# SomeBottle/LinearProgramming

Hardware: AMD Instinct MI355X
Metric: Simplex pivots/sec + HBM GB/s fraction, dense m=16384×n=32768 fp64, 1/2/4/8 GPU (higher is better)
Workload: dtype f64

## Files before the change

### linearprogramming_amd/csrc/lpg_ctx.hip

```cpp
#include <hip/hip_runtime.h>
#include <rccl/rccl.h>

#include <dlfcn.h>
#include <unistd.h>
#include <math.h>
#include <stdarg.h>
#include <stdio.h>
#include <stdlib.h>
#include <string.h>

#include <algorithm>
#include <vector>

#include "../../include/lpg.h"
#include "lpg_internal.h"

using namespace lpg;

namespace {

thread_local char g_err[512];

struct TimingRing {
    std::vector<hipEvent_t> ev;
// ... 205 lines not shown
        const RcclApi *R = rccl_api();
        ncclResult_t r = R->AllReduce(buf, buf, count, ncclFloat64, ncclSum, c->nccl, c->stream);
        if (r != ncclSuccess) return fail(c, LPG_ERR_COMM, "ncclAllReduce: %s", R->GetErrorString(r));
        return 0;
    }
    if (!c->have_hops) return fail(c, LPG_ERR_STATE, "world > 1 but no communicator attached");
    c->hsend.resize(count * sizeof(double));
    HIPCHK(c, hipMemcpyAsync(c->hsend.data(), buf, count * sizeof(double), hipMemcpyDeviceToHost, c->stream));
    HIPCHK(c, hipStreamSynchronize(c->stream));
    if (c->hops.allreduce_sum_f64(c->hops.user, (double *)c->hsend.data(), count) != 0)
        return fail(c, LPG_ERR_COMM, "host allreduce callback failed");
    HIPCHK(c, hipMemcpyAsync(buf, c->hsend.data(), count * sizeof(double), hipMemcpyHostToDevice, c->stream));
    HIPCHK(c, hipStreamSynchronize(c->stream));
    return 0;
}


static int timing_flush(lpg_ctx *c) {
    TimingRing &t = c->tr;
    if (t.used == 0) return 0;
    HIPCHK(c, hipStreamSynchronize(c->stream));
    for (int q = 0; q < t.used; q++) {
        float a = 0, b = 0;
        HIPCHK(c, hipEventElapsedTime(&a, t.ev[3 * q], t.ev[3 * q + 1]));
        HIPCHK(c, hipEventElapsedTime(&b, t.ev[3 * q + 1], t.ev[3 * q + 2]));
        if (t.upd[q] != 2) t.select_ms += a;
        if (t.upd[q]) {
            t.update_ms += b;
            t.count++;
        } else {
            t.select_ms += b;
        }
    }
    t.used = 0;
    return 0;
}

static int timing_mark(lpg_ctx *c, int which, int updated = 1) {
    TimingRing &t = c->tr;
    if (which == 0 && t.used * 3 + 3 > (int)t.ev.size()) {
        int rc = timing_flush(c);
        if (rc) return rc;
    }
    HIPCHK(c, hipEventRecord(t.ev[3 * t.used + which], c->stream));
    if (which == 2) t.upd[t.used++] = (char)updated;
    return 0;
}


static Defer defer_of(const lpg_ctx *c, int q) {
    Defer d;
    d.Pbuf = c->Pbuf;
    d.Cbuf = c->Cbuf;
    d.cs = c->cs;
    d.rq = c->rq;
    d.rqg = c->rqg;
    d.basis = c->basis;
    d.logk = c->logk;
    d.logr = c->logr;
    d.zrow = c->zrow;
    d.kq = c->kq;
    d.lv = c->lv;
    d.colmap = c->colmap;
// ... 17 lines not shown
        case 5: {
            HIPCHK(c, hipStreamSynchronize(c->stream));
            int64_t np = 0;
            HIPCHK(c, hipMemcpy(&np, &c->st->npend, sizeof np, hipMemcpyDeviceToHost));
            np += 1;
            HIPCHK(c, hipMemcpy(&c->st->npend, &np, sizeof np, hipMemcpyHostToDevice));
            break;
        }
        default: break;
    }
    return 0;
}

#endif

static int flush_launch(lpg_ctx *c) {
    int rc;
    const bool re = reorders(c);
#ifdef LPG_TEST_HOOKS
    if (c->inject_flush >= 0 && c->nflush == c->inject_flush && (rc = inject_pending_fault(c))) return rc;
#endif
    c->nflush++;
    const int unit = (c->block_region && c->reg_valid && c->move_unit) ? 1 : 0;
    if (launch_swap_plan(lau(c), geo(c), c->st, defer_of(c, 0), c->colmap, c->inv, c->pairs, re ? 1 : 0, c->defer_k) ||
        (re && launch_move_cols(lau(c), geo(c), c->st, defer_of(c, 0), c->pairs, unit)))
        return fail(c, LPG_ERR_DEVICE, "swap plan launch failed");
#ifdef LPG_TEST_HOOKS
    if (c->inject_rbad >= 0 && c->nflush == c->inject_rbad + 1)
        HIPCHK(c, hipMemsetAsync(&c->st->rbad, 0x01, sizeof(uint32_t), c->stream));
#endif
    if (c->timing && ((rc = timing_mark(c, 0)) || (rc = timing_mark(c, 1)))) return rc;
    const int32_t *tl = (c->block_region && c->reg_valid && re && c->tlive_on && c->skip) ? c->tlive : nullptr;
    c->block_region = false;
    if (launch_flush_main(lau(c), geo(c), c->st, defer_of(c, 0), c->pend, c->skip, c->flush_variant, c->flush_xcd, tl))
        return fail(c, LPG_ERR_DEVICE, "flush launch failed");
    if (c->timing && (rc = timing_mark(c, 2, 2))) return rc;
    if (launch_flush_tail(lau(c), geo(c), c->st, defer_of(c, 0), c->pend, !re))
        return fail(c, LPG_ERR_DEVICE, "flush launch failed");
    if (re) {
        const Defer D = defer_of(c, 0);
        if (launch_fill_cols(lau(c), geo(c), c->pairs, c->st, &D, flush_kmax_supported(c->defer_k),
                             c->reg ? c->bcol0 : nullptr))
            return fail(c, LPG_ERR_DEVICE, "fill launch failed");
        c->permuted = true;
    }
    c->pend = 0;
    return 0;
}

static int materialize(lpg_ctx *c) {
    if (c->defer_k == 0 || c->pend == 0) return 0;
    return flush_launch(c);
}

static int canonicalize(lpg_ctx *c) {
    int rc = materialize(c);
    c->reg_valid = false;
    if (rc || !c->permuted) return rc;
    const int64_t rows = c->nloc + c->nobj;
    if (!c->tmp) {
        c->tmp_rows = std::min<int64_t>(rows, 512);
        HIPCHK(c, hipMalloc(&c->tmp, (size_t)c->tmp_rows * c->ld * sizeof(double)));
    }
    const Geo g = geo(c);
    for (int64_t i0 = 0; i0 < rows; i0 += c->tmp_rows) {
        const int64_t nr = std::min(c->tmp_rows, rows - i0);
        if (launch_gather_rows(lau(c), g, c->inv, c->tmp, i0, nr)) return fail(c, LPG_ERR_DEVICE, "gather launch failed");
// ... 1498 lines not shown
```

### linearprogramming_amd/csrc/lpg_internal.h

```cpp
#pragma once
#include <stddef.h>
#include <stdint.h>

namespace lpg {

constexpr int kBlock = 256;
constexpr int kMaxSelBlocks = 512;
#ifndef LPG_DEFER_MAX
#define LPG_DEFER_MAX 128
#endif

enum : int32_t { RUNNING = 0, OPTIMAL = 1, UNBOUNDED = 2, INFEASIBLE = 3, ITER_LIMIT = 4, NUMERIC = 5 };
enum : int { RULE_DANTZIG = 0, RULE_BLAND = 1 };

struct Slot {
    int64_t k;
    int64_t r;
    int32_t status;
    int32_t pad0;
    int64_t dpend;
};

struct DevState {
    Slot    slot[2];
    int64_t pivots;
    int64_t last_k, last_r;
    int64_t logcap;
    unsigned long long touched;
    unsigned long long work[2];
    int64_t npend;
    unsigned long long fwork;
    int64_t stall;
    int64_t stall_info[4];
    uint32_t rcnt;
    uint32_t rdec;
    uint32_t rbad;
    uint32_t pad1;
    unsigned long long gwork[8];
};
constexpr int64_t kStallResidency = 4;
constexpr int64_t kStallPending = 5;
constexpr int64_t kStallRegion = 6;
constexpr int64_t kNoSlot = INT64_MIN;

struct Defer {
    double  *Pbuf;
    double  *Cbuf;
    int64_t  cs;
    int64_t *rq;
    int64_t *rqg;
    int64_t *basis, *logk, *logr;
    const double *zrow;
    int64_t *kq, *lv;
    const int32_t *colmap;
    const int32_t *inv;
    double  *mul;
    double  *pv;
    int      q;
    int      on;
};
// ... 72 lines not shown
int block_records_bytes(int nwg);
int block_geometry(const Geo &g, int ks, int cus, int want, int *nwg, int *cw, int *rw, size_t *lds);
struct RegionGeo {
    int nwg, cw, rw, nsp, cwx;
    size_t lds;
};
struct RegionArgs {
    const int32_t *live;
    int64_t nlive;
    const int64_t *bcol0;
    int nsp, cwx;
};
int block_geometry_region(const Geo &g, int ks, int cus, int want, int64_t nlive, RegionGeo *out);
int launch_region_build(const Launch &L, const Geo &g, DevState *st, const int64_t *basis, const int32_t *inv,
                        int32_t *mark, int32_t *live, int64_t *bcol0, int64_t nlive, int32_t *tlive);
int launch_region_check(const Launch &L, const Geo &g, const int64_t *basis, const int32_t *inv, int *ok);
int launch_pivot_block(const Launch &L, const Geo &g, int rule, DevState *st, int s0, int q0, int n, Cand *part,
                       int ncand, const Cand *cin, int ncin, const double *Cs0, double *Cs1, const Defer &D,
                       void *rec, uint32_t tag0, int nwg, int cw, int rw, int ks, size_t lds, uint32_t cl,
                       const Xch *X = nullptr, uint32_t xtag0 = 0, const RegionArgs *R = nullptr);
int launch_flush(const Launch &L, const Geo &g, DevState *st, const Defer &D, int kmax, int skip, int which);
int launch_flush_main(const Launch &L, const Geo &g, DevState *st, const Defer &D, int kmax, int skip, int which,
                      int xcd = -1, const int32_t *tlive = nullptr);
int launch_flush_tail(const Launch &L, const Geo &g, DevState *st, const Defer &D, int kmax, bool reset = true);
__host__ __device__ inline int64_t flush_tail_rows(int64_t rows, int64_t nloc) {
    return (rows > 0 && nloc >= 8 * rows && rows >= 64) ? rows / 4 : 0;
}
__host__ __device__ inline int64_t flush_nitems(int64_t ntiles, int64_t rows, int64_t nloc) {
    const int64_t tr = flush_tail_rows(rows, nloc);
    if (rows < 0) rows = -rows;
    if (!tr) return ntiles * ((nloc + rows - 1) / rows);
    const int64_t t0 = ((nloc + rows - 1) / rows - 2) * rows;
    return ntiles * (t0 / rows) + ntiles * ((nloc - t0 + tr - 1) / tr);
}
__host__ __device__ inline void flush_item(int64_t item, int64_t ntiles, int64_t rows, int64_t nloc, int64_t &tile,
                                           int64_t &i0, int64_t &i1) {
    const int64_t tr = flush_tail_rows(rows, nloc);
    if (rows < 0) rows = -rows;
    const int64_t t0 = tr ? ((nloc + rows - 1) / rows - 2) * rows : nloc;
    const int64_t nbig = ntiles * (t0 / rows);
    tile = item % ntiles;
    if (!tr || item < nbig) {
        i0 = (item / ntiles) * rows;
        i1 = i0 + rows;
    } else {
        i0 = t0 + ((item - nbig) / ntiles) * tr;
        i1 = i0 + tr;
// ... 37 lines not shown
                                            int64_t &i0, int64_t &i1) {
    const int h = g % f.H;
    int64_t j;
    const int64_t full = (G.nsb - 1) * G.ntg;
    const int64_t base = G.r0 + (G.nsb - 1) * f.rs;
    if (it < full) {
        j = G.ntg - 1 - it % G.ntg;
        i0 = G.r0 + (it / G.ntg) * f.rs;
        i1 = i0 + f.rs;
    } else if (it - full < G.ntg - G.ttg) {
        j = G.ntg - 1 - (it - full);
        i0 = base;
        i1 = G.r1;
    } else {
        const int64_t k = it - full - (G.ntg - G.ttg);
        j = G.ttg - 1 - k / G.nq;
        i0 = base + (k % G.nq) * G.qrows;
        i1 = i0 + G.qrows;
    }
    if (i1 > G.r1) i1 = G.r1;
    tile = h + (int64_t)f.H * j;
}
int flush_kmax_supported(int k);
int launch_swap_plan(const Launch &L, const Geo &g, DevState *st, const Defer &D, int32_t *colmap, int32_t *inv,
                     int32_t *pairs, int plan, int kmax);
constexpr int kPairW = 4;
int launch_move_cols(const Launch &L, const Geo &g, const DevState *st, const Defer &D, const int32_t *pairs,
                     int unit);
int launch_fill_cols(const Launch &L, const Geo &g, const int32_t *pairs, DevState *st = nullptr,
                     const Defer *D = nullptr, int kmax = 0, int64_t *bcol0 = nullptr);
int launch_gather_rows(const Launch &L, const Geo &g, const int32_t *inv, double *tmp, int64_t i0, int64_t nr);
int launch_iota(const Launch &L, int32_t *a, int64_t n);
int launch_update(const Launch &L, const Geo &g, DevState *st, int s, const double *P, const double *Cs,
                  int64_t *basis, int64_t *logk, int64_t *logr, int variant, int skip);

int launch_dual_rows(const Launch &L, const Geo &g, Cand *part, int nsel);
int launch_dual_row_d(const Launch &L, const Geo &g, DevState *st, int s, const Cand *rc, int nrc, Cand *cp,
                      double *R, const double *Pprev, const double *Cprev, const Defer &D, bool mr);
int launch_dual_ratio(const Launch &L, const Geo &g, const DevState *st, int s, const double *R, Cand *cp);
int launch_dual_col_d(const Launch &L, const Geo &g, DevState *st, int s, const Cand *cp, const double *R, double *Cs,
                      Cand *rc, int nrc_out, const Defer &D);
int launch_dual_pivot(const Launch &L, const Geo &g, DevState *st, int s, Cand *part, int nsel, PricePart *pp,
                      int *pc, int npp, int skip, double *P, double *Cs, bool price_only = false);

#ifdef LPG_PHASES
int debug_phases(unsigned long long *out, int reset);
int debug_block_phases(unsigned long long *out);
#endif
int price_blocks(const Geo &g);
int update_variants();
int update_auto_variant(const Geo &g);

}
// ... 1 lines not shown
```

### linearprogramming_amd/csrc/lpg_kernels.hip

```cpp
#include <hip/hip_runtime.h>
#include <math.h>

#include <stddef.h>
#include <stdlib.h>

#include <algorithm>

#include "lpg_internal.h"
#include "lpg_device.h"
#include "lpg_flushw.h"

namespace lpg {



static inline uint64_t splitmix64_host(uint64_t x) {
    uint64_t z = x + 0x9E3779B97F4A7C15ull;
    z = (z ^ (z >> 30)) * 0xBF58476D1CE4E5B9ull;
    z = (z ^ (z >> 27)) * 0x94D049BB133111EBull;
    return z ^ (z >> 31);
}
static inline uint64_t subkey(uint64_t seed, uint64_t which) {
    return splitmix64_host(seed ^ (which * 0xD1B54A32D192ED03ull));
}
// ... 1534 lines not shown
                for (int r = 0; r < 4; r++) {
                    const int64_t row = i + lk + 4 * r;
                    if (ok[pp] && row < i1) {
                        d2 *dst = (d2 *)(T + row * ld + c0 + 32 * pp + 2 * lc);
                        const d2 v = d2{ae[r], ao[r]};
                        if (NT) __builtin_nontemporal_store(v, dst);
                        else *dst = v;
                    }
                }
            }
            if (!more) break;
            i += 16;
#pragma unroll
            for (int pp = 0; pp < NPAIR; pp++)
#pragma unroll
                for (int r = 0; r < 4; r++) t[pp][r] = tn[pp][r];
        }
    }
    if (threadIdx.x == 0 && touched) atomicAdd(&st->touched, touched);
}


template <int K>
__global__ __launch_bounds__(kBlock) void k_flush_pivot_rows(double *__restrict__ T, Geo g,
                                                             const DevState *__restrict__ st,
                                                             const double *__restrict__ Pbuf,
                                                             const double *__restrict__ mul,
                                                             const int64_t *__restrict__ rq) {
    static_assert((K == 64 || K == 96 || K == 128) && K <= LPG_DEFER_MAX && kBlock == 256,
                  "4 waves x K/16 groups of 4 rows");
    constexpr bool LM = K == 64;
    constexpr int PW = K / (kBlock / 64);
    constexpr int MT = LM ? K * K / kBlock : 1;
    __shared__ double sP[K][64];
    __shared__ __attribute__((aligned(32))) double sM[LM ? K * K : 4];
    __shared__ __attribute__((aligned(32))) double sMg[LM ? 1 : kBlock / 64][LM ? 1 : K][4];
    const int np = (int)st->npend;
    if (np <= 0) return;
    const int c = threadIdx.x & 63, w = threadIdx.x >> 6;
    const int64_t j = (int64_t)blockIdx.x * 64 + c;
    const bool ok = j < g.ncols;
    {
        double v[PW], m[MT];
#pragma unroll
        for (int k = 0; k < PW; k++) {
            const int u = w + 4 * k;
            v[k] = (ok && u < np) ? Pbuf[(int64_t)u * g.ld + j] : 0.0;
        }
#pragma unroll
        for (int k = 0; k < MT; k++) {
            const int e = threadIdx.x + kBlock * k;
            m[k] = (LM && e / K < np) ? mul[(e / K) * LPG_DEFER_MAX + e % K] : 0.0;
        }
#pragma unroll
        for (int k = 0; k < PW; k++) sP[w + 4 * k][c] = v[k];
        if (LM) {
#pragma unroll
            for (int k = 0; k < MT; k++) sM[threadIdx.x + kBlock * k] = m[k];
        }
    }
    const int64_t ru = c < np ? rq[c] : -1;
    const int64_t ru1 = K > 64 && 64 + c < np ? rq[64 + c] : -1;
    __syncthreads();
#pragma unroll 1
    for (int k = 0; k < K / 16; k++) {
        const int grp = (k & 1) ? 8 * (k >> 1) + 7 - w : 8 * (k >> 1) + w;
        const int q0 = 4 * grp;
        if (q0 >= np) continue;
        double x0 = sP[q0][c], x1 = sP[q0 + 1][c], x2 = sP[q0 + 2][c], x3 = sP[q0 + 3][c];
        if (!LM) {
#pragma unroll
            for (int k = 0; k < (LM ? 1 : (K + 63) / 64); k++) {
                const int u = c + 64 * k;
                if (u < K) {
                    const d4 m = *(const d4 *)(mul + (u < np ? u : 0) * LPG_DEFER_MAX + q0);
                    *(d4 *)&sMg[LM ? 0 : w][LM ? 0 : u][0] = u < np ? m : d4{0.0, 0.0, 0.0, 0.0};
                }
            }
        }
        auto m4 = [&](int u) {
            return LM ? *(const d4 *)(sM + u * K + q0) : *(const d4 *)&sMg[LM ? 0 : w][LM ? 0 : u][0];
        };
        if (q0 + 1 < np) {
            const double p = sP[q0 + 1][c];
            const d4 m = m4(q0 + 1);
            x0 = fma(m[0], p, x0);
// ... 9 lines not shown
            const d4 m = m4(q0 + 3);
            x0 = fma(m[0], p, x0);
            x1 = fma(m[1], p, x1);
            x2 = fma(m[2], p, x2);
        }
#pragma unroll 2
        for (int u = q0 + 4; u < np; u++) {
            const double p = sP[u][c];
            const d4 m = m4(u);
            x0 = fma(m[0], p, x0);
            x1 = fma(m[1], p, x1);
            x2 = fma(m[2], p, x2);
            x3 = fma(m[3], p, x3);
        }
        const double xs[4] = {x0, x1, x2, x3};
#pragma unroll
        for (int i = 0; i < 4; i++) {
            const int q = q0 + i;
            if (q >= np) break;
            const int64_t r = q < 64 ? (int64_t)rdl64((uint64_t)ru, q) : (int64_t)rdl64((uint64_t)ru1, q - 64);
            if (r < 0) continue;
            if (__ballot(c > q && ru == r)) continue;
            if (K > 64 && __ballot(64 + c > q && ru1 == r)) continue;
            if (ok) T[r * g.ld + j] = xs[i];
        }
    }
}


constexpr int kMulBlocks = 8;
constexpr int kPlanNT = LPG_DEFER_MAX;
__global__ __launch_bounds__(kPlanNT) void k_swap_plan(DevState *__restrict__ st, const int64_t *__restrict__ kq,
                                                  const int64_t *__restrict__ lv, const int64_t *__restrict__ rq,
                                                  const double *__restrict__ Cbuf, int64_t cs,
                                                  int32_t *__restrict__ colmap, int32_t *__restrict__ inv,
                                                  int32_t *__restrict__ pairs, double *__restrict__ mul, int plan,
                                                  const double *__restrict__ pv, int64_t nloc, int64_t ncols, int kmax) {
    const int64_t np64 = st->npend;
    const bool npbad = np64 < 0 || np64 > kmax;
    const int np = npbad ? 0 : (int)np64;
    {
        const int q = threadIdx.x;
        int what = npbad ? 1 : 0;
        int64_t val = np64;
        if (!npbad && q < np) {
            const int64_t x = plan ? kq[q] : 1, y = plan ? lv[q] : 1, r = rq[q];
            if (x < 1 || x >= ncols) what = 2, val = x;
            else if (y < 1 || y >= ncols) what = 3, val = y;
            else if (r < -1 || r >= nloc) what = 4, val = r;
        }
        __shared__ int first;
        if (q == 0) first = kPlanNT;
        __syncthreads();
        if (what) atomicMin(&first, q);
        if (__syncthreads_or(what != 0)) {
            if (blockIdx.x == 0 && q == first) {
                if (st->stall == 0) {
                    st->stall_info[0] = what;
                    st->stall_info[1] = q;
                    st->stall_info[2] = val;
                    st->stall_info[3] = np64;
                    st->stall = kStallPending;
                }
                st->npend = 0;
                if (pairs) pairs[0] = 0;
                for (int u = 0; u < 2; u++)
                    if (st->slot[u].status == RUNNING) st->slot[u].status = NUMERIC;
            }
            return;
        }
    }
    if (blockIdx.x > 0) {
        constexpr int UB = LPG_DEFER_MAX / kMulBlocks;
        const int q = threadIdx.x;
        const int u0 = (blockIdx.x - 1) * UB;
        const int64_t r = q < np ? rq[q] : -1;
        double v[UB];
#pragma unroll
        for (int k = 0; k < UB; k++) {
            const int u = u0 + k;
            const bool on = u > q && u < np && r >= 0;
            const double c = Cbuf[(int64_t)(on ? u : 0) * cs + (on ? r : 0)];
            v[k] = on ? -c : 0.0;
        }
#pragma unroll
        for (int k = 0; k < UB; k++)
            if (u0 + k < np) mul[(u0 + k) * LPG_DEFER_MAX + q] = v[k];
        return;
    }
    if (!plan) return;
    const int q = threadIdx.x;
    const int64_t x = q < np ? kq[q] : -1, y = q < np ? lv[q] : -1, rx = q < np ? rq[q] : -1;
    const bool pos = q >= np || pv[q] > 0.0;
    __shared__ int64_t sx[kPlanNT], sy[kPlanNT];
    sx[q] = x;
    sy[q] = y;
    bool inE = q < np, inL = q < np;
    int fx = q, fy = q;
    bool fxe = true, fye = false;
    const bool allpos = __syncthreads_count(!pos) == 0;
    if (q == 0 && np > 0 && !allpos) st->rbad = 1;
#pragma unroll 8
    for (int u = 0; u < np; u++) {
        const int64_t a = sx[u], b = sy[u];
        if (u > q) {
            if (a == x || b == x) inE = false;
            if (a == y || b == y) inL = false;
        } else if (u < q) {
            if (a == x && u < fx) { fx = u; fxe = true; }
            if (b == x && u < fx) { fx = u; fxe = false; }
            if (a == y && u < fy) { fy = u; fye = true; }
            if (b == y && u < fy) { fy = u; fye = false; }
        }
    }
    inE = inE && fxe && allpos;
    inL = inL && !fye && allpos;
    constexpr int NW = kPlanNT / 64;
    const int lane = q & 63, wv = q >> 6;
    const unsigned long long me = __ballot(inE), ml = __ballot(inL);
    __shared__ int cE[NW], cL[NW];
    if (lane == 0) {
        cE[wv] = __popcll(me);
        cL[wv] = __popcll(ml);
    }
    __syncthreads();
    int oE = 0, oL = 0, n = 0;
#pragma unroll
    for (int w = 0; w < NW; w++) {
        oE += w < wv ? cE[w] : 0;
        oL += w < wv ? cL[w] : 0;
        n += cE[w];
    }
    const unsigned long long below = (lane == 0) ? 0ull : (~0ull >> (64 - lane));
    const int ie = oE + __popcll(me & below), il = oL + __popcll(ml & below);
    __shared__ int64_t eE[kPlanNT], eL[kPlanNT], eR[kPlanNT], eRL[kPlanNT];
    if (inE) {
        eE[ie] = x;
        eR[ie] = rx;
    }
    if (inL) {
        eL[il] = y;
        eRL[il] = rx;
    }
    __syncthreads();
    if (q < n) {
        const int64_t ce = eE[q], cl = eL[q];
        const int32_t a = inv[ce], b = inv[cl];
        pairs[1 + kPairW * q] = a;
        pairs[2 + kPairW * q] = b;
        pairs[3 + kPairW * q] = (int32_t)eR[q];
        pairs[4 + kPairW * q] = (int32_t)eRL[q];
        colmap[a] = (int32_t)cl;
        colmap[b] = (int32_t)ce;
        inv[cl] = a;
        inv[ce] = b;
    }
    if (q == 0) pairs[0] = n;
}

__global__ __launch_bounds__(kBlock) void k_move_cols(double *__restrict__ T, Geo g, const DevState *__restrict__ st,
                                                      double *__restrict__ Pbuf, const int32_t *__restrict__ pairs,
                                                      int npb, int unit) {
    const int n = pairs[0];
    if (n == 0) return;
    const int nrb = (int)gridDim.x - npb;
    if ((int)blockIdx.x >= nrb) {
        const int np = (int)st->npend;
        const int nt = npb * (int)gridDim.y * kBlock;
        for (int e = (((int)blockIdx.x - nrb) * (int)gridDim.y + (int)blockIdx.y) * kBlock + threadIdx.x; e < np * n;
             e += nt) {
            const int q = e / n, p = e - q * n;
            double *Pq = Pbuf + (int64_t)q * g.ld;
            const int32_t a = pairs[1 + kPairW * p], b = pairs[2 + kPairW * p];
            Pq[a] = Pq[b];
            Pq[b] = 0.0;
        }
        return;
    }
    const int64_t i = (int64_t)blockIdx.x * kBlock + threadIdx.x;
    if (i >= g.nloc + g.nobj) return;
    const bool obj = i >= g.nloc;
    double *row = T + i * g.ld;
    for (int p0 = 16 * blockIdx.y; p0 < n; p0 += 16 * gridDim.y) {
        double va[16], vb[16];
        int ia[16], ib[16], rl[16];
#pragma unroll
        for (int u = 0; u < 16; u++) {
            ia[u] = p0 + u < n ? pairs[1 + kPairW * (p0 + u)] : 0;
            ib[u] = p0 + u < n ? pairs[2 + kPairW * (p0 + u)] : 0;
            rl[u] = p0 + u < n ? pairs[4 + kPairW * (p0 + u)] : -1;
        }
#pragma unroll
        for (int u = 0; u < 16; u++) {
            vb[u] = (unit && !obj) ? ((int64_t)rl[u] == i ? 1.0 : 0.0) : row[ib[u]];
            va[u] = obj ? row[ia[u]] : 0.0;
        }
#pragma unroll
        for (int u = 0; u < 16; u++)
            if (p0 + u < n) {
                row[ia[u]] = vb[u];
                if (obj) row[ib[u]] = va[u];
            }
    }
}

__device__ __forceinline__ void end_block(DevState *st, const Defer &D, int kmax, bool spare_zero = false,
                                          int64_t ld = 0) {
    const int q = threadIdx.x;
    if (spare_zero) {
        const int64_t L = q < kmax ? D.lv[q] : 0;
        if (L > 0) {
            double *col = D.Pbuf + D.inv[L];
            for (int u = 0; u < kmax; u++) col[(int64_t)u * ld] = 0.0;
        }
        __syncthreads();
    }
    if (q == 0) {
        st->npend = 0;
        st->fwork = 0;
    }
    if (q < 8) st->gwork[q] = 0;
    for (int u = q; u < kmax; u += blockDim.x) {
        D.rq[u] = kNoSlot;
        if (D.kq) D.kq[u] = 0;
        if (D.lv) D.lv[u] = 0;
    }
}

__global__ __launch_bounds__(kBlock) void k_end_block(DevState *__restrict__ st, Defer D, int kmax) {
    end_block(st, D, kmax);
}

__global__ __launch_bounds__(kBlock) void k_fill_cols(double *__restrict__ T, Geo g, const int32_t *__restrict__ pairs,
                                                      DevState *__restrict__ st, Defer D, int kmax,
                                                      int64_t *__restrict__ bcol0) {
    if (st && blockIdx.x == 0 && blockIdx.y == 0) end_block(st, D, kmax, bcol0 != nullptr, g.ld);
    if (bcol0 && blockIdx.y == 0) {
        for (int64_t r = (int64_t)blockIdx.x * kBlock + threadIdx.x; r < g.m; r += (int64_t)gridDim.x * kBlock) {
            const int64_t v = D.basis[r];
            bcol0[r] = (v << 32) | (int64_t)(uint32_t)D.inv[v];
        }
    }
    const int n = pairs[0];
    const int64_t i = (int64_t)blockIdx.x * kBlock + threadIdx.x;
    if (i >= g.nloc || n == 0) return;
    double *row = T + i * g.ld;
    for (int p = blockIdx.y; p < n; p += gridDim.y)
        row[pairs[2 + kPairW * p]] = (i == (int64_t)pairs[3 + kPairW * p]) ? 1.0 : 0.0;
}

int launch_swap_plan(const Launch &L, const Geo &g, DevState *st, const Defer &D, int32_t *colmap, int32_t *inv,
                     int32_t *pairs, int plan, int kmax) {
    kmax = flush_kmax_supported(kmax);
    if (!kmax || (plan && !pairs)) return -1;
    hipLaunchKernelGGL(k_swap_plan, dim3(1 + kMulBlocks), dim3(kPlanNT), 0, (hipStream_t)L.stream, st, D.kq, D.lv, D.rq,
                       D.Cbuf, D.cs, colmap, inv, pairs, D.mul, plan, D.pv, g.nloc, g.ncols, kmax);
    return hipGetLastError() == hipSuccess ? 0 : -1;
}

int launch_move_cols(const Launch &L, const Geo &g, const DevState *st, const Defer &D, const int32_t *pairs,
                     int unit) {
    const int64_t rows = g.nloc + g.nobj;
    const int npb = (LPG_DEFER_MAX * LPG_DEFER_MAX + 4 * kBlock - 1) / (4 * kBlock);
    hipLaunchKernelGGL(k_move_cols, dim3((unsigned)((rows + kBlock - 1) / kBlock + npb), 4), dim3(kBlock), 0,
                       (hipStream_t)L.stream, g.T, g, st, D.Pbuf, pairs, npb, unit);
    return hipGetLastError() == hipSuccess ? 0 : -1;
}

int launch_fill_cols(const Launch &L, const Geo &g, const int32_t *pairs, DevState *st, const Defer *D, int kmax,
                     int64_t *bcol0) {
    if (st && (!D || !D->rq || kmax < 1 || kmax > LPG_DEFER_MAX)) return -1;
    if (bcol0 && (!st || !D->basis || !D->inv || !D->lv || !D->Pbuf)) return -1;
    hipLaunchKernelGGL(k_fill_cols, dim3((unsigned)std::max<int64_t>((g.nloc + kBlock - 1) / kBlock, 1), 4), dim3(kBlock),
                       0, (hipStream_t)L.stream, g.T, g, pairs, st, D ? *D : Defer{}, kmax, bcol0);
    return hipGetLastError() == hipSuccess ? 0 : -1;
}

__global__ __launch_bounds__(kBlock) void k_gather_rows(const double *__restrict__ T, Geo g,
                                                        const int32_t *__restrict__ inv, double *__restrict__ tmp,
                                                        int64_t i0, int64_t nr) {
    const int64_t r = blockIdx.y;
    if (r >= nr) return;
    const double *src = T + (i0 + r) * g.ld;
    double *dst = tmp + r * g.ld;
    for (int64_t j = (int64_t)blockIdx.x * kBlock + threadIdx.x; j < g.ncols; j += (int64_t)gridDim.x * kBlock)
        dst[j] = src[inv[j]];
}

int launch_gather_rows(const Launch &L, const Geo &g, const int32_t *inv, double *tmp, int64_t i0, int64_t nr) {
    const int64_t tiles = std::min<int64_t>((g.ncols + kBlock - 1) / kBlock, 64);
    hipLaunchKernelGGL(k_gather_rows, dim3((unsigned)tiles, (unsigned)nr), dim3(kBlock), 0, (hipStream_t)L.stream,
                       g.T, g, inv, tmp, i0, nr);
    return hipGetLastError() == hipSuccess ? 0 : -1;
}

__global__ void k_iota(int32_t *a, int64_t n) {
    for (int64_t j = (int64_t)blockIdx.x * blockDim.x + threadIdx.x; j < n; j += (int64_t)gridDim.x * blockDim.x)
        a[j] = (int32_t)j;
}

int launch_iota(const Launch &L, int32_t *a, int64_t n) {
    hipLaunchKernelGGL(k_iota, dim3(256), dim3(kBlock), 0, (hipStream_t)L.stream, a, n);
    return hipGetLastError() == hipSuccess ? 0 : -1;
}

int flush_kmax_supported(int k) {
    if (k <= 8) return 8;
    if (k <= 16) return 16;
    if (k <= 32) return 32;
    if (k <= 64) return 64;
    if (k <= 96) return 96;
    if (k <= 128 && k <= LPG_DEFER_MAX) return 128;
    return 0;
}

static_assert(offsetof(DevState, fwork) == offsetof(DevState, npend) + sizeof(int64_t),
              "launch_flush clears npend and fwork with one memset");

int launch_flush_tail(const Launch &L, const Geo &g, DevState *st, const Defer &D, int kmax, bool reset) {
    kmax = flush_kmax_supported(kmax);
    if (!kmax) return -1;
    hipStream_t stream = (hipStream_t)L.stream;
    const int64_t ntiles_p = (g.ncols + 63) / 64;
#ifdef LPG_PIVROWS96
    if (kmax == 96)
        hipLaunchKernelGGL(k_flush_pivot_rows<96>, dim3((unsigned)ntiles_p), dim3(kBlock), 0, stream, g.T, g, st,
                           D.Pbuf, D.mul, D.rq);
    else
#endif
    if (kmax > 64)
        hipLaunchKernelGGL(k_flush_pivot_rows<128>, dim3((unsigned)ntiles_p), dim3(kBlock), 0, stream, g.T, g, st,
                           D.Pbuf, D.mul, D.rq);
    else
        hipLaunchKernelGGL(k_flush_pivot_rows<64>, dim3((unsigned)ntiles_p), dim3(kBlock), 0, stream, g.T, g, st,
                           D.Pbuf, D.mul, D.rq);
    if (hipGetLastError() != hipSuccess) return -1;
    if (!reset) return 0;
    hipLaunchKernelGGL(k_end_block, dim3(1), dim3(kBlock), 0, stream, st, D, kmax);
    return hipGetLastError() == hipSuccess ? 0 : -1;
}

int launch_flush(const Launch &L, const Geo &g, DevState *st, const Defer &D, int kmax, int skip, int variant) {
    int rc = launch_swap_plan(L, g, st, D, nullptr, nullptr, nullptr, 0, kmax);
    if (!rc) rc = launch_flush_main(L, g, st, D, kmax, skip, variant);
    return rc ? rc : launch_flush_tail(L, g, st, D, kmax);
}

static bool flush_tail_on() {
    static const int on = [] {
        const char *v = getenv("LPG_FLUSH_TAIL");
        return v ? atoi(v) != 0 : 1;
    }();
    return on != 0;
}

static int64_t flush_rows_env(int64_t def) {
    static const int64_t v = [] {
        const char *e = getenv("LPG_FLUSH_ROWS");
        const long r = e ? atol(e) : 0;
        return (int64_t)((r >= 64 && r <= 8192 && r % 64 == 0) ? r : 0);
    }();
    return v ? v : def;
}

static int64_t flush_minitems_env(int64_t def) {
    static const int64_t v = [] {
// ... 115 lines not shown
```

Before: 31540.

## Fuse swap plan with column move, and pivot rows with fill and end_block

On the reordering flush path, the swap-plan and column-move kernels are merged into one block_trade kernel. The pivot-row update, column fill, bcol0 build and end_block are merged into a single block_finish kernel, which uses a last-arrival atomic counter (the new ecnt field) so the final block runs end_block. This removes several kernel launches and their serialization per flush. In exchange it adds an atomic grid-completion handshake and a per-tile ballot scan over the swap pairs so pivot-row writes skip columns that fill_cols will overwrite.

```diff
diff --git a/linearprogramming_amd/csrc/lpg_ctx.hip b/linearprogramming_amd/csrc/lpg_ctx.hip
--- a/linearprogramming_amd/csrc/lpg_ctx.hip
+++ b/linearprogramming_amd/csrc/lpg_ctx.hip
@@ -251,9 +251,11 @@
     HIPCHK(c, hipStreamSynchronize(c->stream));
     for (int q = 0; q < t.used; q++) {
         float a = 0, b = 0;
-        HIPCHK(c, hipEventElapsedTime(&a, t.ev[3 * q], t.ev[3 * q + 1]));
+        if (t.upd[q] != 2) {
+            HIPCHK(c, hipEventElapsedTime(&a, t.ev[3 * q], t.ev[3 * q + 1]));
+            t.select_ms += a;
+        }
         HIPCHK(c, hipEventElapsedTime(&b, t.ev[3 * q + 1], t.ev[3 * q + 2]));
-        if (t.upd[q] != 2) t.select_ms += a;
         if (t.upd[q]) {
             t.update_ms += b;
             t.count++;
@@ -267,7 +269,7 @@
 
 static int timing_mark(lpg_ctx *c, int which, int updated = 1) {
     TimingRing &t = c->tr;
-    if (which == 0 && t.used * 3 + 3 > (int)t.ev.size()) {
+    if ((which == 0 || (which == 1 && updated == 2)) && t.used * 3 + 3 > (int)t.ev.size()) {
         int rc = timing_flush(c);
         if (rc) return rc;
     }
@@ -331,27 +333,26 @@
 #endif
     c->nflush++;
     const int unit = (c->block_region && c->reg_valid && c->move_unit) ? 1 : 0;
-    if (launch_swap_plan(lau(c), geo(c), c->st, defer_of(c, 0), c->colmap, c->inv, c->pairs, re ? 1 : 0, c->defer_k) ||
-        (re && launch_move_cols(lau(c), geo(c), c->st, defer_of(c, 0), c->pairs, unit)))
+    if (re ? launch_block_trade(lau(c), geo(c), c->st, defer_of(c, 0), c->colmap, c->inv, c->pairs, c->defer_k, unit)
+           : launch_swap_plan(lau(c), geo(c), c->st, defer_of(c, 0), c->defer_k))
         return fail(c, LPG_ERR_DEVICE, "swap plan launch failed");
 #ifdef LPG_TEST_HOOKS
     if (c->inject_rbad >= 0 && c->nflush == c->inject_rbad + 1)
         HIPCHK(c, hipMemsetAsync(&c->st->rbad, 0x01, sizeof(uint32_t), c->stream));
 #endif
-    if (c->timing && ((rc = timing_mark(c, 0)) || (rc = timing_mark(c, 1)))) return rc;
+    if (c->timing && (rc = timing_mark(c, 1, 2))) return rc;
     const int32_t *tl = (c->block_region && c->reg_valid && re && c->tlive_on && c->skip) ? c->tlive : nullptr;
     c->block_region = false;
     if (launch_flush_main(lau(c), geo(c), c->st, defer_of(c, 0), c->pend, c->skip, c->flush_variant, c->flush_xcd, tl))
         return fail(c, LPG_ERR_DEVICE, "flush launch failed");
     if (c->timing && (rc = timing_mark(c, 2, 2))) return rc;
-    if (launch_flush_tail(lau(c), geo(c), c->st, defer_of(c, 0), c->pend, !re))
+    if (re) {
+        if (launch_block_finish(lau(c), geo(c), c->st, defer_of(c, 0), c->pairs, c->pend, c->defer_k,
+                                c->reg ? c->bcol0 : nullptr))
+            return fail(c, LPG_ERR_DEVICE, "flush launch failed");
+        c->permuted = true;
+    } else if (launch_flush_tail(lau(c), geo(c), c->st, defer_of(c, 0), c->pend)) {
         return fail(c, LPG_ERR_DEVICE, "flush launch failed");
-    if (re) {
-        const Defer D = defer_of(c, 0);
-        if (launch_fill_cols(lau(c), geo(c), c->pairs, c->st, &D, flush_kmax_supported(c->defer_k),
-                             c->reg ? c->bcol0 : nullptr))
-            return fail(c, LPG_ERR_DEVICE, "fill launch failed");
-        c->permuted = true;
     }
     c->pend = 0;
     return 0;
diff --git a/linearprogramming_amd/csrc/lpg_internal.h b/linearprogramming_amd/csrc/lpg_internal.h
--- a/linearprogramming_amd/csrc/lpg_internal.h
+++ b/linearprogramming_amd/csrc/lpg_internal.h
@@ -35,7 +35,7 @@
     uint32_t rcnt;
     uint32_t rdec;
     uint32_t rbad;
-    uint32_t pad1;
+    uint32_t ecnt;
     unsigned long long gwork[8];
 };
 constexpr int64_t kStallResidency = 4;
@@ -154,7 +154,7 @@
 int launch_flush(const Launch &L, const Geo &g, DevState *st, const Defer &D, int kmax, int skip, int which);
 int launch_flush_main(const Launch &L, const Geo &g, DevState *st, const Defer &D, int kmax, int skip, int which,
                       int xcd = -1, const int32_t *tlive = nullptr);
-int launch_flush_tail(const Launch &L, const Geo &g, DevState *st, const Defer &D, int kmax, bool reset = true);
+int launch_flush_tail(const Launch &L, const Geo &g, DevState *st, const Defer &D, int kmax);
 __host__ __device__ inline int64_t flush_tail_rows(int64_t rows, int64_t nloc) {
     return (rows > 0 && nloc >= 8 * rows && rows >= 64) ? rows / 4 : 0;
 }
@@ -238,13 +238,12 @@
     tile = h + (int64_t)f.H * j;
 }
 int flush_kmax_supported(int k);
-int launch_swap_plan(const Launch &L, const Geo &g, DevState *st, const Defer &D, int32_t *colmap, int32_t *inv,
-                     int32_t *pairs, int plan, int kmax);
 constexpr int kPairW = 4;
-int launch_move_cols(const Launch &L, const Geo &g, const DevState *st, const Defer &D, const int32_t *pairs,
-                     int unit);
-int launch_fill_cols(const Launch &L, const Geo &g, const int32_t *pairs, DevState *st = nullptr,
-                     const Defer *D = nullptr, int kmax = 0, int64_t *bcol0 = nullptr);
+int launch_block_trade(const Launch &L, const Geo &g, DevState *st, const Defer &D, int32_t *colmap, int32_t *inv,
+                       int32_t *pairs, int kmax, int unit);
+int launch_block_finish(const Launch &L, const Geo &g, DevState *st, const Defer &D, const int32_t *pairs, int pend,
+                        int kmax, int64_t *bcol0);
+int launch_swap_plan(const Launch &L, const Geo &g, DevState *st, const Defer &D, int kmax);
 int launch_gather_rows(const Launch &L, const Geo &g, const int32_t *inv, double *tmp, int64_t i0, int64_t nr);
 int launch_iota(const Launch &L, int32_t *a, int64_t n);
 int launch_update(const Launch &L, const Geo &g, DevState *st, int s, const double *P, const double *Cs,
diff --git a/linearprogramming_amd/csrc/lpg_kernels.hip b/linearprogramming_amd/csrc/lpg_kernels.hip
--- a/linearprogramming_amd/csrc/lpg_kernels.hip
+++ b/linearprogramming_amd/csrc/lpg_kernels.hip
@@ -1580,11 +1580,10 @@
 
 
 template <int K>
-__global__ __launch_bounds__(kBlock) void k_flush_pivot_rows(double *__restrict__ T, Geo g,
-                                                             const DevState *__restrict__ st,
-                                                             const double *__restrict__ Pbuf,
-                                                             const double *__restrict__ mul,
-                                                             const int64_t *__restrict__ rq) {
+__device__ __forceinline__ double *pivot_rows_tile(double *__restrict__ T, const Geo &g,
+                                                   const DevState *__restrict__ st, const double *__restrict__ Pbuf,
+                                                   const double *__restrict__ mul, const int64_t *__restrict__ rq,
+                                                   int64_t tile, const int32_t *__restrict__ pairs, bool run = true) {
     static_assert((K == 64 || K == 96 || K == 128) && K <= LPG_DEFER_MAX && kBlock == 256,
                   "4 waves x K/16 groups of 4 rows");
     constexpr bool LM = K == 64;
@@ -1593,11 +1592,25 @@
     __shared__ double sP[K][64];
     __shared__ __attribute__((aligned(32))) double sM[LM ? K * K : 4];
     __shared__ __attribute__((aligned(32))) double sMg[LM ? 1 : kBlock / 64][LM ? 1 : K][4];
+    if (!run) return &sP[0][0];
     const int np = (int)st->npend;
-    if (np <= 0) return;
+    if (np <= 0) return &sP[0][0];
     const int c = threadIdx.x & 63, w = threadIdx.x >> 6;
-    const int64_t j = (int64_t)blockIdx.x * 64 + c;
+    const int64_t j = tile * 64 + c;
     const bool ok = j < g.ncols;
+    unsigned long long skip = 0ull;
+    if (pairs) {
+        const int n = pairs[0];
+        for (int p0 = 0; p0 < n; p0 += 64) {
+            const int64_t off = p0 + c < n ? (int64_t)pairs[2 + kPairW * (p0 + c)] - tile * 64 : -1;
+            unsigned long long hit = __ballot(off >= 0 && off < 64);
+            while (hit) {
+                const int l = __ffsll((long long)hit) - 1;
+                skip |= 1ull << __shfl((int)off, l, 64);
+                hit &= hit - 1;
+            }
+        }
+    }
     {
         double v[PW], m[MT];
 #pragma unroll
@@ -1620,6 +1633,7 @@
     const int64_t ru = c < np ? rq[c] : -1;
     const int64_t ru1 = K > 64 && 64 + c < np ? rq[64 + c] : -1;
     __syncthreads();
+    const bool wr = ok && !((skip >> c) & 1ull);
 #pragma unroll 1
     for (int k = 0; k < K / 16; k++) {
         const int grp = (k & 1) ? 8 * (k >> 1) + 7 - w : 8 * (k >> 1) + w;
@@ -1675,84 +1689,126 @@
             if (r < 0) continue;
             if (__ballot(c > q && ru == r)) continue;
             if (K > 64 && __ballot(64 + c > q && ru1 == r)) continue;
-            if (ok) T[r * g.ld + j] = xs[i];
-        }
-    }
+            if (wr) T[r * g.ld + j] = xs[i];
+        }
+    }
+    return &sP[0][0];
+}
+
+template <int K>
+__global__ __launch_bounds__(kBlock) void k_flush_pivot_rows(double *__restrict__ T, Geo g,
+                                                             const DevState *__restrict__ st,
+                                                             const double *__restrict__ Pbuf,
+                                                             const double *__restrict__ mul,
+                                                             const int64_t *__restrict__ rq) {
+    pivot_rows_tile<K>(T, g, st, Pbuf, mul, rq, (int64_t)blockIdx.x, nullptr);
 }
 
 
 constexpr int kMulBlocks = 8;
 constexpr int kPlanNT = LPG_DEFER_MAX;
-__global__ __launch_bounds__(kPlanNT) void k_swap_plan(DevState *__restrict__ st, const int64_t *__restrict__ kq,
-                                                  const int64_t *__restrict__ lv, const int64_t *__restrict__ rq,
-                                                  const double *__restrict__ Cbuf, int64_t cs,
-                                                  int32_t *__restrict__ colmap, int32_t *__restrict__ inv,
-                                                  int32_t *__restrict__ pairs, double *__restrict__ mul, int plan,
-                                                  const double *__restrict__ pv, int64_t nloc, int64_t ncols, int kmax) {
+
+__device__ __forceinline__ bool pending_refused(DevState *__restrict__ st, const int64_t *__restrict__ kq,
+                                                const int64_t *__restrict__ lv, const int64_t *__restrict__ rq,
+                                                int32_t *pairs, bool plan, bool record, int64_t nloc, int64_t ncols,
+                                                int kmax, int &np_out) {
     const int64_t np64 = st->npend;
     const bool npbad = np64 < 0 || np64 > kmax;
     const int np = npbad ? 0 : (int)np64;
-    {
-        const int q = threadIdx.x;
-        int what = npbad ? 1 : 0;
-        int64_t val = np64;
-        if (!npbad && q < np) {
-            const int64_t x = plan ? kq[q] : 1, y = plan ? lv[q] : 1, r = rq[q];
-            if (x < 1 || x >= ncols) what = 2, val = x;
-            else if (y < 1 || y >= ncols) what = 3, val = y;
-            else if (r < -1 || r >= nloc) what = 4, val = r;
-        }
-        __shared__ int first;
-        if (q == 0) first = kPlanNT;
-        __syncthreads();
-        if (what) atomicMin(&first, q);
-        if (__syncthreads_or(what != 0)) {
-            if (blockIdx.x == 0 && q == first) {
-                if (st->stall == 0) {
-                    st->stall_info[0] = what;
-                    st->stall_info[1] = q;
-                    st->stall_info[2] = val;
-                    st->stall_info[3] = np64;
-                    st->stall = kStallPending;
-                }
-                st->npend = 0;
-                if (pairs) pairs[0] = 0;
-                for (int u = 0; u < 2; u++)
-                    if (st->slot[u].status == RUNNING) st->slot[u].status = NUMERIC;
-            }
-            return;
-        }
-    }
-    if (blockIdx.x > 0) {
-        constexpr int UB = LPG_DEFER_MAX / kMulBlocks;
-        const int q = threadIdx.x;
-        const int u0 = (blockIdx.x - 1) * UB;
-        const int64_t r = q < np ? rq[q] : -1;
-        double v[UB];
-#pragma unroll
-        for (int k = 0; k < UB; k++) {
-            const int u = u0 + k;
-            const bool on = u > q && u < np && r >= 0;
-            const double c = Cbuf[(int64_t)(on ? u : 0) * cs + (on ? r : 0)];
-            v[k] = on ? -c : 0.0;
-        }
-#pragma unroll
-        for (int k = 0; k < UB; k++)
-            if (u0 + k < np) mul[(u0 + k) * LPG_DEFER_MAX + q] = v[k];
-        return;
-    }
-    if (!plan) return;
+    np_out = np;
+    const int q = threadIdx.x;
+    int what = npbad ? 1 : 0;
+    int64_t val = np64;
+    if (!npbad && q < np) {
+        const int64_t x = plan ? kq[q] : 1, y = plan ? lv[q] : 1, r = rq[q];
+        if (x < 1 || x >= ncols) what = 2, val = x;
+        else if (y < 1 || y >= ncols) what = 3, val = y;
+        else if (r < -1 || r >= nloc) what = 4, val = r;
+    }
+    __shared__ int first;
+    if (q == 0) first = (int)blockDim.x;
+    __syncthreads();
+    if (what) atomicMin(&first, q);
+    if (!__syncthreads_or(what != 0)) return false;
+    if (record && q == first) {
+        if (st->stall == 0) {
+            st->stall_info[0] = what;
+            st->stall_info[1] = q;
+            st->stall_info[2] = val;
+            st->stall_info[3] = np64;
+            st->stall = kStallPending;
+        }
+        st->npend = 0;
+        if (pairs) pairs[0] = 0;
+        for (int u = 0; u < 2; u++)
+            if (st->slot[u].status == RUNNING) st->slot[u].status = NUMERIC;
+    }
+    return true;
+}
+
+__device__ __forceinline__ void build_mul(int blk, int np, const int64_t *__restrict__ rq,
+                                          const double *__restrict__ Cbuf, int64_t cs, double *__restrict__ mul) {
+    constexpr int UB = LPG_DEFER_MAX / kMulBlocks;
+    const int q = threadIdx.x;
+    if (q >= kPlanNT) return;
+    const int u0 = blk * UB;
+    const int64_t r = q < np ? rq[q] : -1;
+    double v[UB];
+#pragma unroll
+    for (int k = 0; k < UB; k++) {
+        const int u = u0 + k;
+        const bool on = u > q && u < np && r >= 0;
+        const double c = Cbuf[(int64_t)(on ? u : 0) * cs + (on ? r : 0)];
+        v[k] = on ? -c : 0.0;
+    }
+#pragma unroll
+    for (int k = 0; k < UB; k++)
+        if (u0 + k < np) mul[(u0 + k) * LPG_DEFER_MAX + q] = v[k];
+}
+
+__global__ __launch_bounds__(kPlanNT) void k_swap_plan(DevState *__restrict__ st, const int64_t *__restrict__ rq,
+                                                  const double *__restrict__ Cbuf, int64_t cs,
+                                                  double *__restrict__ mul, int64_t nloc, int64_t ncols, int kmax) {
+    int np;
+    if (pending_refused(st, nullptr, nullptr, rq, nullptr, false, blockIdx.x == 0, nloc, ncols, kmax, np)) return;
+    if (blockIdx.x > 0) build_mul((int)blockIdx.x - 1, np, rq, Cbuf, cs, mul);
+}
+
+__device__ __forceinline__ bool last_arrival(uint32_t *cnt, uint32_t nwg, uint32_t *ticket) {
+    asm volatile("s_waitcnt vmcnt(0) lgkmcnt(0)" ::: "memory");
+    __syncthreads();
+    if (threadIdx.x == 0) {
+        *ticket = atomicAdd(cnt, 1u);
+        if (*ticket == nwg - 1) atomicExch(cnt, 0u);
+    }
+    __syncthreads();
+    return *ticket == nwg - 1;
+}
+
+struct TradePlan {
+    int64_t eE[kPlanNT], eL[kPlanNT];
+    int32_t a[kPlanNT], b[kPlanNT];
+    int32_t r[kPlanNT], rl[kPlanNT];
+    int n, allpos;
+};
+
+template <int NT>
+__device__ __forceinline__ void trade_plan(TradePlan &tp, int np, const int64_t *__restrict__ kq,
+                                           const int64_t *__restrict__ lv, const int64_t *__restrict__ rq,
+                                           const double *__restrict__ pv, const int32_t *inv) {
+    static_assert(NT >= kPlanNT && NT % 64 == 0, "one thread per event");
     const int q = threadIdx.x;
     const int64_t x = q < np ? kq[q] : -1, y = q < np ? lv[q] : -1, rx = q < np ? rq[q] : -1;
     const bool pos = q >= np || pv[q] > 0.0;
     __shared__ int64_t sx[kPlanNT], sy[kPlanNT];
-    sx[q] = x;
-    sy[q] = y;
+    if (q < kPlanNT) {
+        sx[q] = x;
+        sy[q] = y;
+    }
     bool inE = q < np, inL = q < np;
     int fx = q, fy = q;
     bool fxe = true, fye = false;
     const bool allpos = __syncthreads_count(!pos) == 0;
-    if (q == 0 && np > 0 && !allpos) st->rbad = 1;
 #pragma unroll 8
     for (int u = 0; u < np; u++) {
         const int64_t a = sx[u], b = sy[u];
@@ -1768,7 +1824,7 @@
     }
     inE = inE && fxe && allpos;
     inL = inL && !fye && allpos;
-    constexpr int NW = kPlanNT / 64;
+    constexpr int NW = NT / 64;
     const int lane = q & 63, wv = q >> 6;
     const unsigned long long me = __ballot(inE), ml = __ballot(inL);
     __shared__ int cE[NW], cL[NW];
@@ -1786,74 +1842,95 @@
     }
     const unsigned long long below = (lane == 0) ? 0ull : (~0ull >> (64 - lane));
     const int ie = oE + __popcll(me & below), il = oL + __popcll(ml & below);
-    __shared__ int64_t eE[kPlanNT], eL[kPlanNT], eR[kPlanNT], eRL[kPlanNT];
     if (inE) {
-        eE[ie] = x;
-        eR[ie] = rx;
+        tp.eE[ie] = x;
+        tp.r[ie] = (int32_t)rx;
     }
     if (inL) {
-        eL[il] = y;
-        eRL[il] = rx;
+        tp.eL[il] = y;
+        tp.rl[il] = (int32_t)rx;
+    }
+    if (q == 0) {
+        tp.n = n;
+        tp.allpos = allpos ? 1 : 0;
     }
     __syncthreads();
     if (q < n) {
-        const int64_t ce = eE[q], cl = eL[q];
-        const int32_t a = inv[ce], b = inv[cl];
+        tp.a[q] = inv[tp.eE[q]];
+        tp.b[q] = inv[tp.eL[q]];
+    }
+    __syncthreads();
+}
+
+__global__ __launch_bounds__(kBlock) void k_block_trade(double *__restrict__ T, Geo g, DevState *st, Defer D,
+                                                        int32_t *colmap, int32_t *inv, int32_t *pairs, int npb,
+                                                        int unit, int kmax) {
+    __shared__ TradePlan tp;
+    int np;
+    const bool bad = pending_refused(st, D.kq, D.lv, D.rq, pairs, true, blockIdx.x == 0 && blockIdx.y == 0, g.nloc,
+                                     g.ncols, kmax, np);
+    if (!bad) {
+        trade_plan<kBlock>(tp, np, D.kq, D.lv, D.rq, D.pv, inv);
+        const int n = tp.n;
+        const int nrb = (int)gridDim.x - npb;
+        if ((int)blockIdx.x >= nrb) {
+            const int pb = ((int)blockIdx.x - nrb) * (int)gridDim.y + (int)blockIdx.y;
+            if (pb < kMulBlocks) build_mul(pb, np, D.rq, D.Cbuf, D.cs, D.mul);
+            const int nt = npb * (int)gridDim.y * kBlock;
+            for (int e = pb * kBlock + threadIdx.x; e < np * n; e += nt) {
+                const int q = e / n, p = e - q * n;
+                double *Pq = D.Pbuf + (int64_t)q * g.ld;
+                const int32_t a = tp.a[p], b = tp.b[p];
+                Pq[a] = Pq[b];
+                Pq[b] = 0.0;
+            }
+        } else {
+            const int64_t i = (int64_t)blockIdx.x * kBlock + threadIdx.x;
+            if (i < g.nloc + g.nobj) {
+                const bool obj = i >= g.nloc;
+                double *row = T + i * g.ld;
+                for (int p0 = 16 * blockIdx.y; p0 < n; p0 += 16 * gridDim.y) {
+                    double va[16], vb[16];
+                    int ia[16], ib[16], rl[16];
+#pragma unroll
+                    for (int u = 0; u < 16; u++) {
+                        ia[u] = p0 + u < n ? tp.a[p0 + u] : 0;
+                        ib[u] = p0 + u < n ? tp.b[p0 + u] : 0;
+                        rl[u] = p0 + u < n ? tp.rl[p0 + u] : -1;
+                    }
+#pragma unroll
+                    for (int u = 0; u < 16; u++) {
+                        vb[u] = (unit && !obj) ? ((int64_t)rl[u] == i ? 1.0 : 0.0) : row[ib[u]];
+                        va[u] = obj ? row[ia[u]] : 0.0;
+                    }
+#pragma unroll
+                    for (int u = 0; u < 16; u++)
+                        if (p0 + u < n) {
+                            row[ia[u]] = vb[u];
+                            if (obj) row[ib[u]] = va[u];
+                        }
+                }
+            }
+        }
+    }
+    __shared__ uint32_t ticket;
+    if (!last_arrival(&st->ecnt, gridDim.x * gridDim.y, &ticket) || bad) return;
+    const int q = threadIdx.x, n = tp.n;
+    if (q < n) {
+        const int64_t ce = tp.eE[q], cl = tp.eL[q];
+        const int32_t a = tp.a[q], b = tp.b[q];
         pairs[1 + kPairW * q] = a;
         pairs[2 + kPairW * q] = b;
-        pairs[3 + kPairW * q] = (int32_t)eR[q];
-        pairs[4 + kPairW * q] = (int32_t)eRL[q];
+        pairs[3 + kPairW * q] = tp.r[q];
+        pairs[4 + kPairW * q] = tp.rl[q];
         colmap[a] = (int32_t)cl;
         colmap[b] = (int32_t)ce;
         inv[cl] = a;
         inv[ce] = b;
     }
-    if (q == 0) pairs[0] = n;
-}
-
-__global__ __launch_bounds__(kBlock) void k_move_cols(double *__restrict__ T, Geo g, const DevState *__restrict__ st,
-                                                      double *__restrict__ Pbuf, const int32_t *__restrict__ pairs,
-                                                      int npb, int unit) {
-    const int n = pairs[0];
-    if (n == 0) return;
-    const int nrb = (int)gridDim.x - npb;
-    if ((int)blockIdx.x >= nrb) {
-        const int np = (int)st->npend;
-        const int nt = npb * (int)gridDim.y * kBlock;
-        for (int e = (((int)blockIdx.x - nrb) * (int)gridDim.y + (int)blockIdx.y) * kBlock + threadIdx.x; e < np * n;
-             e += nt) {
-            const int q = e / n, p = e - q * n;
-            double *Pq = Pbuf + (int64_t)q * g.ld;
-            const int32_t a = pairs[1 + kPairW * p], b = pairs[2 + kPairW * p];
-            Pq[a] = Pq[b];
-            Pq[b] = 0.0;
-        }
-        return;
-    }
-    const int64_t i = (int64_t)blockIdx.x * kBlock + threadIdx.x;
-    if (i >= g.nloc + g.nobj) return;
-    const bool obj = i >= g.nloc;
-    double *row = T + i * g.ld;
-    for (int p0 = 16 * blockIdx.y; p0 < n; p0 += 16 * gridDim.y) {
-        double va[16], vb[16];
-        int ia[16], ib[16], rl[16];
-#pragma unroll
-        for (int u = 0; u < 16; u++) {
-            ia[u] = p0 + u < n ? pairs[1 + kPairW * (p0 + u)] : 0;
-            ib[u] = p0 + u < n ? pairs[2 + kPairW * (p0 + u)] : 0;
-            rl[u] = p0 + u < n ? pairs[4 + kPairW * (p0 + u)] : -1;
-        }
-#pragma unroll
-        for (int u = 0; u < 16; u++) {
-            vb[u] = (unit && !obj) ? ((int64_t)rl[u] == i ? 1.0 : 0.0) : row[ib[u]];
-            va[u] = obj ? row[ia[u]] : 0.0;
-        }
-#pragma unroll
-        for (int u = 0; u < 16; u++)
-            if (p0 + u < n) {
-                row[ia[u]] = vb[u];
-                if (obj) row[ib[u]] = va[u];
-            }
+    if (q == 0) {
+        pairs[0] = n;
+        if (np > 0 && !tp.allpos) st->rbad = 1;
     }
 }
 
@@ -1884,48 +1961,66 @@
     end_block(st, D, kmax);
 }
 
-__global__ __launch_bounds__(kBlock) void k_fill_cols(double *__restrict__ T, Geo g, const int32_t *__restrict__ pairs,
-                                                      DevState *__restrict__ st, Defer D, int kmax,
-                                                      int64_t *__restrict__ bcol0) {
-    if (st && blockIdx.x == 0 && blockIdx.y == 0) end_block(st, D, kmax, bcol0 != nullptr, g.ld);
-    if (bcol0 && blockIdx.y == 0) {
-        for (int64_t r = (int64_t)blockIdx.x * kBlock + threadIdx.x; r < g.m; r += (int64_t)gridDim.x * kBlock) {
-            const int64_t v = D.basis[r];
-            bcol0[r] = (v << 32) | (int64_t)(uint32_t)D.inv[v];
-        }
-    }
-    const int n = pairs[0];
-    const int64_t i = (int64_t)blockIdx.x * kBlock + threadIdx.x;
-    if (i >= g.nloc || n == 0) return;
-    double *row = T + i * g.ld;
-    for (int p = blockIdx.y; p < n; p += gridDim.y)
-        row[pairs[2 + kPairW * p]] = (i == (int64_t)pairs[3 + kPairW * p]) ? 1.0 : 0.0;
-}
-
-int launch_swap_plan(const Launch &L, const Geo &g, DevState *st, const Defer &D, int32_t *colmap, int32_t *inv,
-                     int32_t *pairs, int plan, int kmax) {
+template <int K>
+__global__ __launch_bounds__(kBlock) void k_block_finish(double *__restrict__ T, Geo g, DevState *st, Defer D,
+                                                         const int32_t *__restrict__ pairs, int kmax,
+                                                         int64_t *__restrict__ bcol0, int ntp, int nrb) {
+    const bool tile = (int)blockIdx.x < ntp;
+    double *lds = pivot_rows_tile<K>(T, g, st, D.Pbuf, D.mul, D.rq, (int64_t)blockIdx.x, pairs, tile);
+    if (!tile) {
+        const int e = (int)blockIdx.x - ntp, bx = e % nrb, by = e / nrb;
+        if (bcol0 && by == 0) {
+            for (int64_t r = (int64_t)bx * kBlock + threadIdx.x; r < g.m; r += (int64_t)nrb * kBlock) {
+                const int64_t v = D.basis[r];
+                bcol0[r] = (v << 32) | (int64_t)(uint32_t)D.inv[v];
+            }
+        }
+        const int n = pairs[0];
+        const int64_t i = (int64_t)bx * kBlock + threadIdx.x;
+        if (i < g.nloc) {
+            double *row = T + i * g.ld;
+            for (int p = by; p < n; p += 4)
+                row[pairs[2 + kPairW * p]] = (i == (int64_t)pairs[3 + kPairW * p]) ? 1.0 : 0.0;
+        }
+    }
+    if (last_arrival(&st->ecnt, gridDim.x, (uint32_t *)lds)) end_block(st, D, kmax, bcol0 != nullptr, g.ld);
+}
+
+int launch_swap_plan(const Launch &L, const Geo &g, DevState *st, const Defer &D, int kmax) {
     kmax = flush_kmax_supported(kmax);
-    if (!kmax || (plan && !pairs)) return -1;
-    hipLaunchKernelGGL(k_swap_plan, dim3(1 + kMulBlocks), dim3(kPlanNT), 0, (hipStream_t)L.stream, st, D.kq, D.lv, D.rq,
-                       D.Cbuf, D.cs, colmap, inv, pairs, D.mul, plan, D.pv, g.nloc, g.ncols, kmax);
+    if (!kmax) return -1;
+    hipLaunchKernelGGL(k_swap_plan, dim3(1 + kMulBlocks), dim3(kPlanNT), 0, (hipStream_t)L.stream, st, D.rq, D.Cbuf,
+                       D.cs, D.mul, g.nloc, g.ncols, kmax);
     return hipGetLastError() == hipSuccess ? 0 : -1;
 }
 
-int launch_move_cols(const Launch &L, const Geo &g, const DevState *st, const Defer &D, const int32_t *pairs,
-                     int unit) {
+int launch_block_trade(const Launch &L, const Geo &g, DevState *st, const Defer &D, int32_t *colmap, int32_t *inv,
+                       int32_t *pairs, int kmax, int unit) {
+    kmax = flush_kmax_supported(kmax);
+    if (!kmax || !pairs || !colmap || !inv || !D.kq || !D.lv || !D.pv) return -1;
     const int64_t rows = g.nloc + g.nobj;
     const int npb = (LPG_DEFER_MAX * LPG_DEFER_MAX + 4 * kBlock - 1) / (4 * kBlock);
-    hipLaunchKernelGGL(k_move_cols, dim3((unsigned)((rows + kBlock - 1) / kBlock + npb), 4), dim3(kBlock), 0,
-                       (hipStream_t)L.stream, g.T, g, st, D.Pbuf, pairs, npb, unit);
+    static_assert(4 * ((LPG_DEFER_MAX * LPG_DEFER_MAX + 4 * kBlock - 1) / (4 * kBlock)) >= kMulBlocks,
+                  "the first kMulBlocks P-entry blocks build mul");
+    hipLaunchKernelGGL(k_block_trade, dim3((unsigned)((rows + kBlock - 1) / kBlock + npb), 4), dim3(kBlock), 0,
+                       (hipStream_t)L.stream, g.T, g, st, D, colmap, inv, pairs, npb, unit, kmax);
     return hipGetLastError() == hipSuccess ? 0 : -1;
 }
 
-int launch_fill_cols(const Launch &L, const Geo &g, const int32_t *pairs, DevState *st, const Defer *D, int kmax,
-                     int64_t *bcol0) {
-    if (st && (!D || !D->rq || kmax < 1 || kmax > LPG_DEFER_MAX)) return -1;
-    if (bcol0 && (!st || !D->basis || !D->inv || !D->lv || !D->Pbuf)) return -1;
-    hipLaunchKernelGGL(k_fill_cols, dim3((unsigned)std::max<int64_t>((g.nloc + kBlock - 1) / kBlock, 1), 4), dim3(kBlock),
-                       0, (hipStream_t)L.stream, g.T, g, pairs, st, D ? *D : Defer{}, kmax, bcol0);
+int launch_block_finish(const Launch &L, const Geo &g, DevState *st, const Defer &D, const int32_t *pairs, int pend,
+                        int kmax, int64_t *bcol0) {
+    pend = flush_kmax_supported(pend);
+    kmax = flush_kmax_supported(kmax);
+    if (!pend || !kmax || !st || !pairs || !D.rq) return -1;
+    if (bcol0 && (!D.basis || !D.inv || !D.lv || !D.Pbuf)) return -1;
+    const int ntp = (int)((g.ncols + 63) / 64);
+    const int nrb = (int)std::max<int64_t>((g.nloc + kBlock - 1) / kBlock, 1);
+    const dim3 grid((unsigned)(ntp + 4 * nrb));
+    hipStream_t stream = (hipStream_t)L.stream;
+    if (pend > 64)
+        hipLaunchKernelGGL(k_block_finish<128>, grid, dim3(kBlock), 0, stream, g.T, g, st, D, pairs, kmax, bcol0, ntp, nrb);
+    else
+        hipLaunchKernelGGL(k_block_finish<64>, grid, dim3(kBlock), 0, stream, g.T, g, st, D, pairs, kmax, bcol0, ntp, nrb);
     return hipGetLastError() == hipSuccess ? 0 : -1;
 }
 
@@ -1970,7 +2065,7 @@
 static_assert(offsetof(DevState, fwork) == offsetof(DevState, npend) + sizeof(int64_t),
               "launch_flush clears npend and fwork with one memset");
 
-int launch_flush_tail(const Launch &L, const Geo &g, DevState *st, const Defer &D, int kmax, bool reset) {
+int launch_flush_tail(const Launch &L, const Geo &g, DevState *st, const Defer &D, int kmax) {
     kmax = flush_kmax_supported(kmax);
     if (!kmax) return -1;
     hipStream_t stream = (hipStream_t)L.stream;
@@ -1988,13 +2083,12 @@
         hipLaunchKernelGGL(k_flush_pivot_rows<64>, dim3((unsigned)ntiles_p), dim3(kBlock), 0, stream, g.T, g, st,
                            D.Pbuf, D.mul, D.rq);
     if (hipGetLastError() != hipSuccess) return -1;
-    if (!reset) return 0;
     hipLaunchKernelGGL(k_end_block, dim3(1), dim3(kBlock), 0, stream, st, D, kmax);
     return hipGetLastError() == hipSuccess ? 0 : -1;
 }
 
 int launch_flush(const Launch &L, const Geo &g, DevState *st, const Defer &D, int kmax, int skip, int variant) {
-    int rc = launch_swap_plan(L, g, st, D, nullptr, nullptr, nullptr, 0, kmax);
+    int rc = launch_swap_plan(L, g, st, D, kmax);
     if (!rc) rc = launch_flush_main(L, g, st, D, kmax, skip, variant);
     return rc ? rc : launch_flush_tail(L, g, st, D, kmax);
 }
```

New measurement: 31500. No clear change (-0.1%).
